# uzh-rpg/rpg_svo

Measured on AMD Instinct MI355X. Metric: frames/sec sparse-align+pose-refine (VGA, 4 pyr lvls); ATE vs CPU ref, higher is better.
Workload: dtype value = default build: K1 f32 pixels/residuals/chi2/per-pixel products, f64 Jacobian rows/partials/reductions/projection/solve/pose; K4 f64 (reference-width build: roofline_f64_build.value)

## Files before the change

### rpg_svo_amd/csrc/sparse_align.hip

```cpp
#include <cstdlib>
#include <map>
#include <mutex>
#include <utility>

#include "sia_common.h"

using namespace svo_capi;
using namespace svo_dev;
using namespace svo_sia;

namespace {

#define MINW(BLOCK) ((BLOCK) >= 256 ? 4 : 3)

#ifdef SIA_PROFILE
#define SIA_T() ((long long)__builtin_readcyclecounter())
#define SIA_ACC(k, t0, t1) prof[k] += (t1) - (t0)
#else
#define SIA_T() 0ll
#define SIA_ACC(k, t0, t1)
#endif

constexpr int MAX_WAVES = SVO_HIP_MAX_PATCHES / 64;

#if defined(SIA_F64_PARTIALS)
using sia_pix = double;
using sia_acc = double;
#undef MINW
#define MINW(BLOCK) 3
#else
using sia_pix = float;
using sia_acc = double;
#endif

struct SplitModel {
  double q[2][4], t[2][3];
};

struct SiaLds {
  SplitModel sm;
  double Rt[12];
  int sw_done, sw_stop, sw_nmeas, sw_cur, sw_old;
  double sw_chi2;
  double H[21];
  double Hinv[36];
  double A[36];
  sia_acc part[2][MAX_WAVES][8];
  int chg[2][MAX_WAVES];
  int xfail;
  sia_acc Hpart[MAX_WAVES][24];
  long long lo[SVO_HIP_MAX_LEVELS];
  int lw[SVO_HIP_MAX_LEVELS];
  int lh[SVO_HIP_MAX_LEVELS];
  int lp[SVO_HIP_MAX_LEVELS];
};
__shared__ SiaLds g_s;


template <int PARTS>
__device__ __forceinline__ void sia_rebuild_hinv(int lane, int nw, [[maybe_unused]] XChunk* xh, [[maybe_unused]] int part,
                                                 [[maybe_unused]] unsigned gen, [[maybe_unused]] int& xfail) {
  asm volatile("" : "+v"(lane));
#ifndef SVO_HOST_MATH_TEST
  if constexpr (PARTS > 1) {
    static_assert((PARTS - 1) * 21 <= 64, "one lane per chunk of the other parts");
    const int j = lane / 21, k = lane - 21 * j;
    double v = 0.0;
    for (int w = 0; w < nw; ++w) v += (double)g_s.Hpart[w][k];
    if (j == 0) sia_xstore(xh + part * SIA_XH_SLOTS + k, v, gen);
    const int other = j < part ? j : j + 1;
    double got = 0.0;
    if (j < PARTS - 1) got = sia_xpoll(xh + other * SIA_XH_SLOTS + k, gen, xfail);
    if (xfail) g_s.xfail = 1;
    double tot = 0.0;
#pragma unroll
    for (int p = 0; p < PARTS; ++p) {
      const double theirs = __shfl(got, (p < part ? p : p - 1) * 21 + k, 64);
      const double term = p == part ? v : theirs;
      tot = p == 0 ? term : tot + term;
    }
    if (lane < 21) g_s.H[lane] = tot;
  } else
#endif
  if (lane < 21) {
    double v = 0.0;
    for (int w = 0; w < nw; ++w) v += (double)g_s.Hpart[w][lane];
    g_s.H[lane] = v;
  }
  SVO_WAVE_LDS_FENCE();
  const int gi = lane / 6, gj = lane - 6 * gi;
  if (lane < 36) {
    g_s.A[lane] = g_s.H[sym6_rt(gi, gj)];
    g_s.Hinv[lane] = (gi == gj) ? 1.0 : 0.0;
  }
  for (int k = 0; k < 6; ++k) {
    SVO_WAVE_LDS_FENCE();
    if (lane < 36) {
      const double p = g_s.A[k * 6 + k];
      const double aik = g_s.A[gi * 6 + k];
      const double akj = g_s.A[k * 6 + gj];
      const double bkj = g_s.Hinv[k * 6 + gj];
      const double aij = g_s.A[lane];
      const double bij = g_s.Hinv[lane];
      const double ip = (fabs(p) > 2.2250738585072014e-308) ? sia_rcp(p) : 0.0;
      const double na = (gi == k) ? akj * ip : aij - aik * (akj * ip);
      const double nb = (gi == k) ? bkj * ip : bij - aik * (bkj * ip);
      SVO_LANES_LDS_FENCE();
      g_s.A[lane] = na;
      g_s.Hinv[lane] = nb;
    }
  }
}


__device__ __forceinline__ float sia_bilerp(float wtl, float wtr, float wbl, float wbr, float tl, float tr, float bl, float br) {
  return __builtin_fmaf(wbr, br, __builtin_fmaf(wbl, bl, __builtin_fmaf(wtr, tr, wtl * tl)));
}
typedef float sia_f2 __attribute__((ext_vector_type(2)));
__device__ __forceinline__ sia_f2 sia_bilerp2(sia_f2 wtl, sia_f2 wtr, sia_f2 wbl, sia_f2 wbr, sia_f2 tl, sia_f2 tr, sia_f2 bl,
                                              sia_f2 br) {
  return __builtin_elementwise_fma(wbr, br, __builtin_elementwise_fma(wbl, bl, __builtin_elementwise_fma(wtr, tr, wtl * tl)));
}

#ifdef SIA_F64_PARTIALS
#define SIA_PACKED 0
#else
#define SIA_PACKED 1
#endif
template <int BLOCK, bool WC, bool DIST, int PARTS = 1>
__global__ void __launch_bounds__(BLOCK, PARTS > 1 ? 1 : ((DIST && BLOCK < 1024) ? 3 : MINW(BLOCK))) sia_kernel(const SiaArgs a) {
  constexpr int NW = BLOCK / 64;
  int b, part = 0;
  if constexpr (PARTS > 1) {
    b = (int)(blockIdx.x / (8 * PARTS)) * 8 + (int)(blockIdx.x % 8);
    part = (int)(blockIdx.x / 8) % PARTS;
    if (b >= a.B) return;
  } else {
    b = (int)xcd_contiguous_block();
  }
  [[maybe_unused]] XChunk* const xbase = PARTS > 1 ? static_cast<XChunk*>(a.xw) + (size_t)b * SIA_X_BLOCK : nullptr;
  [[maybe_unused]] unsigned xseq = 0;
#ifndef SVO_HOST_MATH_TEST
  if constexpr (PARTS > 1) xseq = (unsigned)__builtin_amdgcn_readfirstlane((int)sia_xload(xbase + SIA_X_CHUNKS).lo);
#endif
  [[maybe_unused]] int xfail = 0;
  const int tid = threadIdx.x;
  const int lane = tid & 63;
  const int wave = tid >> 6;

  __shared__ float4 s_bt[8][BLOCK];

  int n = a.n[b];
  n = n > a.n_stride ? a.n_stride : n;
  const svo_hip_sia_params P = a.P;

  if (n <= 0) {
    if (tid == 0 && part == 0) {
      for (int k = 0; k < 12; ++k) a.T_out[12 * b + k] = a.T_in[12 * b + k];
      if (a.H_out)
        for (int k = 0; k < 36; ++k) a.H_out[36 * b + k] = 0.0;
      a.n_tracked[b] = 0;
      if (a.iters)
        for (int k = 0; k < SVO_HIP_MAX_LEVELS; ++k) a.iters[SVO_HIP_MAX_LEVELS * b + k] = 0;
      if (a.chi2) a.chi2[b] = 1e10;
      if (a.status) a.status[b] = 0;
    }
    return;
  }

  const int pid = part * BLOCK + tid;
  const size_t fo = (size_t)b * a.n_stride + pid;
  const bool has = (pid < n) && (a.valid ? a.valid[fo] != 0 : true);
  double X = 0, Y = 0, Z = 1;
  if (has) {
    X = a.xyz[3 * fo];
    Y = a.xyz[3 * fo + 1];
    Z = a.xyz[3 * fo + 2];
  }
  double px_kept0 = 0, px_kept1 = 0;
  if (has) {
    px_kept0 = a.px[2 * fo];
    px_kept1 = a.px[2 * fo + 1];
  }
  const double rz = sia_rcp(Z);
  const sia_acc zi = (sia_acc)rz;
  const sia_acc xn = (sia_acc)(X * rz);
  const sia_acc yn = (sia_acc)(Y * rz);
  const uint8_t* ref_base = a.store + (int64_t)a.ref_slot[b] * a.L.slot_bytes;
  const uint8_t* cur_base = a.store + (int64_t)a.cur_slot[b] * a.L.slot_bytes;

  if (tid == 0) {
#pragma unroll
    for (int k = 0; k < SVO_HIP_MAX_LEVELS; ++k) {
      g_s.lw[k] = a.L.w[k];
      g_s.lh[k] = a.L.h[k];
      g_s.lp[k] = a.L.pitch[k];
      g_s.lo[k] = a.L.offset[k];
    }
    for (int k = 0; k < 21; ++k) g_s.H[k] = 0.0;
    g_s.xfail = 0;
    if (a.iters && part == 0)
      for (int k = 0; k < SVO_HIP_MAX_LEVELS; ++k) a.iters[SVO_HIP_MAX_LEVELS * b + k] = 0;
  }
  double R[9], tr[3];
  {
    double q[4];
    for (int k = 0; k < 9; ++k) R[k] = a.T_in[12 * b + k];
    for (int k = 0; k < 3; ++k) tr[k] = a.T_in[12 * b + 9 + k];
    quat_from_R(R, q);
    quat_to_R(q, R);
    if (tid == 0) {
      for (int k = 0; k < 4; ++k) g_s.sm.q[0][k] = q[k];
      for (int k = 0; k < 3; ++k) g_s.sm.t[0][k] = tr[k];
    }
  }
  int m_cur = 0, m_old = 0;
  double chi2_prev = 1e10;
  int stop = 0;
  int n_meas_last = 0;
  int buf = 0;

  const int sw = (NW > 1) ? (int)(blockIdx.x % NW) : 0;
  sia_pix Sxx = 0, Sxy = 0, Syy = 0;
  sia_acc gmask = 0;
  bool vis = false;

  __syncthreads();

#ifdef SIA_PROFILE
  long long prof[8] = {0, 0, 0, 0, 0, 0, 0, 0};
  const long long t_begin = SIA_T();
#endif
  for (int level = P.max_level; level >= P.min_level; --level) {
    [[maybe_unused]] const long long tl0 = SIA_T();
    const int cols = g_s.lw[level], rows = g_s.lh[level], pitch = g_s.lp[level];
    const uint8_t* ref_img = ref_base + g_s.lo[level];
    const uint8_t* cur_img = cur_base + g_s.lo[level];
    const float scale = pow2_inv_f32(level);
    const sia_acc fl = (sia_acc)(fabs(P.fx) * pow2_inv_f64(level));

    uint32_t wc[WC ? 7 : 1][3];
    int wc_u0 = 0, wc_v0 = -100000;
    if (WC) {
#pragma unroll
      for (int r = 0; r < (WC ? 7 : 1); ++r) wc[r][0] = wc[r][1] = wc[r][2] = 0u;
    }
    {
      const double pxx = px_kept0, pxy = px_kept1;
      const float u_ref = (float)(pxx * (double)scale);
      const float v_ref = (float)(pxy * (double)scale);
      const int u_i = (int)floorf(u_ref);
      const int v_i = (int)floorf(v_ref);
      const bool inb = has && !(u_i - 3 < 0 || v_i - 3 < 0 || u_i + 3 >= cols || v_i + 3 >= rows);
      Sxx = Sxy = Syy = 0;
      if (inb) {
        vis = true;
        gmask = 1;
        const float su = u_ref - (float)u_i, sv = v_ref - (float)v_i;
        const float wtl = (1.f - su) * (1.f - sv);
        const float wtr = su * (1.f - sv);
        const float wbl = (1.f - su) * sv;
        const float wbr = su * sv;
        float Bt[6][6];
        float Wp[7], Wc[7];
        uint32_t rw[7][3];
        const int rxa = run_start(u_i - 3, 7);
        const uint32_t rbo = (uint32_t)(u_i - 3 - rxa);
        load_window12<7>(ref_img, pitch, rxa, v_i - 3, rw);
        cut_row7(rw[0], rbo, Wp);
#pragma unroll
        for (int r = 0; r < 6; ++r) {
          cut_row7(rw[r + 1], rbo, Wc);
#pragma unroll
          for (int c = 0; c < 6; ++c) {
            const bool need = ((r >= 1 && r <= 4)) || ((c >= 1 && c <= 4));
            if (need) Bt[r][c] = sia_bilerp(wtl, wtr, wbl, wbr, Wp[c], Wp[c + 1], Wc[c], Wc[c + 1]);
          }
#pragma unroll
          for (int c = 0; c < 7; ++c) Wp[c] = Wc[c];
        }
#pragma unroll
        for (int y = 0; y < 4; ++y)
#pragma unroll
          for (int x = 0; x < 4; ++x) {
            const float dx = 0.5f * (Bt[y + 1][x + 2] - Bt[y + 1][x]);
            const float dy = 0.5f * (Bt[y + 2][x + 1] - Bt[y][x + 1]);
            Sxx += (sia_pix)dx * (sia_pix)dx;
            Sxy += (sia_pix)dx * (sia_pix)dy;
            Syy += (sia_pix)dy * (sia_pix)dy;
          }
#if SIA_PACKED
        s_bt[0][tid] = make_float4(Bt[0][1], Bt[0][3], Bt[0][2], Bt[0][4]);
        s_bt[1][tid] = make_float4(Bt[1][0], Bt[1][2], Bt[1][1], Bt[1][3]);
        s_bt[2][tid] = make_float4(Bt[1][4], Bt[1][5], Bt[2][0], Bt[2][2]);
        s_bt[3][tid] = make_float4(Bt[2][1], Bt[2][3], Bt[2][4], Bt[2][5]);
        s_bt[4][tid] = make_float4(Bt[3][0], Bt[3][2], Bt[3][1], Bt[3][3]);
        s_bt[5][tid] = make_float4(Bt[3][4], Bt[3][5], Bt[4][0], Bt[4][2]);
        s_bt[6][tid] = make_float4(Bt[4][1], Bt[4][3], Bt[4][4], Bt[4][5]);
        s_bt[7][tid] = make_float4(Bt[5][1], Bt[5][3], Bt[5][2], Bt[5][4]);
#else
        s_bt[0][tid] = make_float4(Bt[0][1], Bt[0][2], Bt[0][3], Bt[0][4]);
        s_bt[1][tid] = make_float4(Bt[1][0], Bt[1][1], Bt[1][2], Bt[1][3]);
        s_bt[2][tid] = make_float4(Bt[1][4], Bt[1][5], Bt[2][0], Bt[2][1]);
        s_bt[3][tid] = make_float4(Bt[2][2], Bt[2][3], Bt[2][4], Bt[2][5]);
        s_bt[4][tid] = make_float4(Bt[3][0], Bt[3][1], Bt[3][2], Bt[3][3]);
        s_bt[5][tid] = make_float4(Bt[3][4], Bt[3][5], Bt[4][0], Bt[4][1]);
        s_bt[6][tid] = make_float4(Bt[4][2], Bt[4][3], Bt[4][4], Bt[4][5]);
        s_bt[7][tid] = make_float4(Bt[5][1], Bt[5][2], Bt[5][3], Bt[5][4]);
#endif
      } else {
        gmask = 0;
      }
    }

    m_old = m_cur;
    int inH = -1;
    int evals = 0;
    SIA_ACC(5, tl0, SIA_T());
    for (int iter = 0; iter < P.n_iter; ++iter) {
      [[maybe_unused]] const long long tp0 = SIA_T();
      bool m = false;
      sia_pix gx = 0, gy = 0;
      float c2 = 0.f;
      if (vis) {
        const double xc = R[0] * X + R[1] * Y + R[2] * Z + tr[0];
        const double yc = R[3] * X + R[4] * Y + R[5] * Z + tr[1];
        const double zc = R[6] * X + R[7] * Y + R[8] * Z + tr[2];
        double izc = __builtin_amdgcn_rcp(zc);
        izc = fma(fma(-zc, izc, 1.0), izc, izc);
        izc = fma(fma(-zc, izc, 1.0), izc, izc);
        double pu, pv;
        if (DIST) {
          Cam cm;
          cm.fx = P.fx; cm.fy = P.fy; cm.cx = P.cx; cm.cy = P.cy;
          cm.width = 0; cm.height = 0;
          cm.model = P.cam_model;
#pragma unroll
          for (int k = 0; k < 5; ++k) cm.d[k] = P.d[k];
          const double uvn[2] = {xc * izc, yc * izc};
          double pxd[2];
          world2cam_uv(cm, uvn, pxd);
          pu = pxd[0];
          pv = pxd[1];
        } else {
          pu = P.fx * (xc * izc) + P.cx;
          pv = P.fy * (yc * izc) + P.cy;
        }
        const float u_cur = (float)pu * scale;
        const float v_cur = (float)pv * scale;
        const float fu = floorf(u_cur), fv = floorf(v_cur);
        if (fu - 3.f >= 0.f && fv - 3.f >= 0.f && fu + 3.f < (float)cols && fv + 3.f < (float)rows) {
          m = true;
          const int u_i = (int)fu, v_i = (int)fv;
          const float su = u_cur - fu, sv = v_cur - fv;
          const float wtl = (1.f - su) * (1.f - sv);
          const float wtr = su * (1.f - sv);
          const float wbl = (1.f - su) * sv;
          const float wbr = su * sv;
          {
#if SIA_PACKED
          typedef float f2 __attribute__((ext_vector_type(2)));
          uint32_t cw[5][3];
          uint32_t cbo = 0;
          uint64_t k0 = 0, k1 = 0, kup = 0;
          int bo = 0;
          if (WC) {
            int r0 = (v_i - 2) - wc_v0;
            bo = (u_i - 2) - wc_u0;
            if (!(r0 >= 0 && r0 <= 2 && bo >= 0 && bo <= 7)) {
              wc_v0 = v_i - 3;
              wc_u0 = run_start(u_i - 3, 7);
              load_window12<(WC ? 7 : 1)>(cur_img, pitch, wc_u0, wc_v0, wc);
              r0 = 1;
              bo = (u_i - 2) - wc_u0;
            }
            k0 = SVO_BALLOT_ACTIVE(r0 == 0);
            k1 = SVO_BALLOT_ACTIVE(r0 == 1);
            kup = SVO_BALLOT_ACTIVE(bo >= 4);
          } else {
            const int cxa = run_start(u_i - 2, 5);
            cbo = (uint32_t)(u_i - 2 - cxa);
            load_window12<5>(cur_img, pitch, cxa, v_i - 2, cw);
          }
#define SIA_WIN_ROW(r, p02, p13, p24)                                                                                   \
  do {                                                                                                                  \
    float o_[5];                                                                                                        \
    if (WC) {                                                                                                           \
      constexpr int S_ = WC ? 1 : 0;                                                                                    \
      const uint32_t d0_ = sel_e64(k0, wc[(r) * S_][0], sel_e64(k1, wc[((r) + 1) * S_][0], wc[((r) + 2) * S_][0]));     \
      const uint32_t d1_ = sel_e64(k0, wc[(r) * S_][1], sel_e64(k1, wc[((r) + 1) * S_][1], wc[((r) + 2) * S_][1]));     \
      const uint32_t d2_ = sel_e64(k0, wc[(r) * S_][2], sel_e64(k1, wc[((r) + 1) * S_][2], wc[((r) + 2) * S_][2]));     \
      cut_row5(d0_, d1_, d2_, bo, kup, o_);                                                                             \
    } else {                                                                                                            \
      cut_row5_plain(cw[WC ? 0 : (r)], cbo, o_);                                                                        \
    }                                                                                                                   \
    p02 = f2{o_[0], o_[2]};                                                                                             \
    p13 = f2{o_[1], o_[3]};                                                                                             \
    p24 = f2{o_[2], o_[4]};                                                                                             \
  } while (0)
          const float2* const bt2 = reinterpret_cast<const float2*>(&s_bt[0][0]);
#define SIA_BT2(q, h) bt2[((q) * BLOCK + tid) * 2 + (h)]
          const f2 vtl = f2{wtl, wtl}, vtr = f2{wtr, wtr}, vbl = f2{wbl, wbl}, vbr = f2{wbr, wbr};
          f2 c2v = f2{0.f, 0.f}, gxv = f2{0.f, 0.f}, gyv = f2{0.f, 0.f};
          f2 t02, t13, t24, b02, b13, b24;
          SIA_WIN_ROW(0, t02, t13, t24);
          SIA_WIN_ROW(1, b02, b13, b24);
          f2 a13, a24, b02t, b13t, b45t, c02, c13, c45;
          { const float2 v0 = SIA_BT2(0, 0), v1 = SIA_BT2(0, 1); a13 = f2{v0.x, v0.y}; a24 = f2{v1.x, v1.y}; }
          { const float2 v0 = SIA_BT2(1, 0), v1 = SIA_BT2(1, 1), v2 = SIA_BT2(2, 0);
            b02t = f2{v0.x, v0.y}; b13t = f2{v1.x, v1.y}; b45t = f2{v2.x, v2.y}; }
          { const float2 v0 = SIA_BT2(2, 1), v1 = SIA_BT2(3, 0), v2 = SIA_BT2(3, 1);
            c02 = f2{v0.x, v0.y}; c13 = f2{v1.x, v1.y}; c45 = f2{v2.x, v2.y}; }
#pragma unroll
          for (int y = 0; y < 4; ++y) {
            f2 n02 = f2{0.f, 0.f}, n13 = f2{0.f, 0.f}, n45 = f2{0.f, 0.f};
            if (y == 0) { const float2 v0 = SIA_BT2(4, 0), v1 = SIA_BT2(4, 1), v2 = SIA_BT2(5, 0);
                          n02 = f2{v0.x, v0.y}; n13 = f2{v1.x, v1.y}; n45 = f2{v2.x, v2.y}; }
            if (y == 1) { const float2 v0 = SIA_BT2(5, 1), v1 = SIA_BT2(6, 0), v2 = SIA_BT2(6, 1);
                          n02 = f2{v0.x, v0.y}; n13 = f2{v1.x, v1.y}; n45 = f2{v2.x, v2.y}; }
            if (y == 2) { const float2 v0 = SIA_BT2(7, 0), v1 = SIA_BT2(7, 1);
                          n13 = f2{v0.x, v0.y}; n45 = f2{v1.x, v1.y}; }
            const f2 b24t = f2{b02t.y, b45t.x}, b35t = f2{b13t.y, b45t.y};
            const f2 c24 = (y < 3) ? f2{c02.y, c45.x} : c45;
            const f2 Ia = sia_bilerp2(vtl, vtr, vbl, vbr, t02, t13, b02, b13);
            const f2 Ib = sia_bilerp2(vtl, vtr, vbl, vbr, t13, t24, b13, b24);
            const f2 ra = Ia - b13t, rb = Ib - b24t;
            c2v += ra * ra;
            c2v += rb * rb;
            gxv += ra * (b24t - b02t);
            gxv += rb * (b35t - b13t);
            gyv += ra * (c13 - a13);
            gyv += rb * (c24 - a24);
            if (y < 3) {
              f2 w02, w13, w24;
              SIA_WIN_ROW(y + 2, w02, w13, w24);
              t02 = b02; t13 = b13; t24 = b24;
              b02 = w02; b13 = w13; b24 = w24;
              a13 = b13t; a24 = b24t;
              b02t = c02; b13t = c13; b45t = c45;
              c02 = n02; c13 = n13; c45 = n45;
              asm volatile("" ::: "memory");
            }
          }
#undef SIA_WIN_ROW
#undef SIA_BT2
          c2 += c2v.x + c2v.y;
          gx += gxv.x + gxv.y;
          gy += gyv.x + gyv.y;
#else
          float W[5][5];
          if (WC) {
            int r0 = (v_i - 2) - wc_v0;
            int bo = (u_i - 2) - wc_u0;
            if (!(r0 >= 0 && r0 <= 2 && bo >= 0 && bo <= 7)) {
              wc_v0 = v_i - 3;
              wc_u0 = run_start(u_i - 3, 7);
              load_window12<(WC ? 7 : 1)>(cur_img, pitch, wc_u0, wc_v0, wc);
              r0 = 1;
              bo = (u_i - 2) - wc_u0;
            }
            const uint64_t k0 = SVO_BALLOT_ACTIVE(r0 == 0), k1 = SVO_BALLOT_ACTIVE(r0 == 1);
            const uint64_t kup = SVO_BALLOT_ACTIVE(bo >= 4);
#pragma unroll
            for (int r = 0; r < 5; ++r) {
              constexpr int S = WC ? 1 : 0;
              const uint32_t d0 = sel_e64(k0, wc[r * S][0], sel_e64(k1, wc[(r + 1) * S][0], wc[(r + 2) * S][0]));
              const uint32_t d1 = sel_e64(k0, wc[r * S][1], sel_e64(k1, wc[(r + 1) * S][1], wc[(r + 2) * S][1]));
              const uint32_t d2 = sel_e64(k0, wc[r * S][2], sel_e64(k1, wc[(r + 1) * S][2], wc[(r + 2) * S][2]));
              cut_row5(d0, d1, d2, bo, kup, W[r]);
            }
          } else {
            uint32_t cw[5][3];
            const int cxa = run_start(u_i - 2, 5);
            const uint32_t cbo = (uint32_t)(u_i - 2 - cxa);
            load_window12<5>(cur_img, pitch, cxa, v_i - 2, cw);
#pragma unroll
            for (int r = 0; r < 5; ++r) cut_row5_plain(cw[r], cbo, W[r]);
          }
          float Bt[6][6];
          {
            const float4 q0 = s_bt[0][tid], q1 = s_bt[1][tid], q2 = s_bt[2][tid], q3 = s_bt[3][tid];
            const float4 q4 = s_bt[4][tid], q5 = s_bt[5][tid], q6 = s_bt[6][tid], q7 = s_bt[7][tid];
            Bt[0][0] = Bt[0][5] = Bt[5][0] = Bt[5][5] = 0.f;
            Bt[0][1] = q0.x; Bt[0][2] = q0.y; Bt[0][3] = q0.z; Bt[0][4] = q0.w;
            Bt[1][0] = q1.x; Bt[1][1] = q1.y; Bt[1][2] = q1.z; Bt[1][3] = q1.w;
            Bt[1][4] = q2.x; Bt[1][5] = q2.y; Bt[2][0] = q2.z; Bt[2][1] = q2.w;
            Bt[2][2] = q3.x; Bt[2][3] = q3.y; Bt[2][4] = q3.z; Bt[2][5] = q3.w;
            Bt[3][0] = q4.x; Bt[3][1] = q4.y; Bt[3][2] = q4.z; Bt[3][3] = q4.w;
            Bt[3][4] = q5.x; Bt[3][5] = q5.y; Bt[4][0] = q5.z; Bt[4][1] = q5.w;
            Bt[4][2] = q6.x; Bt[4][3] = q6.y; Bt[4][4] = q6.z; Bt[4][5] = q6.w;
            Bt[5][1] = q7.x; Bt[5][2] = q7.y; Bt[5][3] = q7.z; Bt[5][4] = q7.w;
          }
#pragma unroll
          for (int y = 0; y < 4; ++y)
#pragma unroll
            for (int x = 0; x < 4; ++x) {
              const float I = sia_bilerp(wtl, wtr, wbl, wbr, W[y][x], W[y][x + 1], W[y + 1][x], W[y + 1][x + 1]);
              const float res = I - Bt[y + 1][x + 1];
              c2 += res * res;
              gx += (sia_pix)res * (sia_pix)(Bt[y + 1][x + 2] - Bt[y + 1][x]);
              gy += (sia_pix)res * (sia_pix)(Bt[y + 2][x + 1] - Bt[y][x + 1]);
            }
#endif
          }
        }
      }
      {
        const sia_acc gsc = (sia_acc)0.5 * fl * gmask;
        const sia_acc gxf = m ? (sia_acc)gx * gsc : (sia_acc)0, gyf = m ? (sia_acc)gy * gsc : (sia_acc)0;
        sia_acc part[8];
        sia_acc zi_ = zi, xn_ = xn, yn_ = yn;
        asm volatile("" : "+v"(zi_), "+v"(xn_), "+v"(yn_));
        part[0] = zi_ * gxf;
        part[1] = zi_ * gyf;
        part[2] = -zi_ * (xn_ * gxf + yn_ * gyf);
        part[3] = -(xn_ * yn_ * gxf + ((sia_acc)1 + yn_ * yn_) * gyf);
        part[4] = ((sia_acc)1 + xn_ * xn_) * gxf + xn_ * yn_ * gyf;
        part[5] = xn_ * gyf - yn_ * gxf;
        part[6] = (sia_acc)c2;
        part[7] = m ? (sia_acc)16 : (sia_acc)0;
        [[maybe_unused]] const long long tp1 = SIA_T();
        SIA_ACC(0, tp0, tp1);
        const sia_acc tot = wave_reduce8(part, lane);
        if ((lane & 7) == 0) g_s.part[buf][wave][lane >> 3] = tot;
        const int mine = __builtin_amdgcn_ballot_w64((int)m != inH) != 0ull;
        if (lane == 0) g_s.chg[buf][wave] = mine;
        SIA_ACC(1, tp1, SIA_T());
      }
      [[maybe_unused]] const long long tb0 = SIA_T();
      __syncthreads();
      int changed = 0;
#pragma unroll
      for (int w = 0; w < NW; ++w) changed |= g_s.chg[buf][w];
      [[maybe_unused]] double xtot = 0.0;
#ifndef SVO_HOST_MATH_TEST
      if constexpr (PARTS > 1) {
        ++xseq;
        const int xp = lane >> 4, xk = lane & 15;
        double own = 0.0;
        if (xk < 8) {
#pragma unroll
          for (int w = 0; w < NW; ++w) own += (double)g_s.part[buf][w][xk];
        } else if (xk == 8) {
          own = (double)changed;
        }
        XChunk* const slot = xbase + (size_t)(xseq & 1) * (SIA_X_MAX_PARTS * SIA_X_SLOTS);
        if (wave == sw && xp == part && xk < 9) sia_xstore(slot + part * SIA_X_SLOTS + xk, own, xseq);
        double val = own;
        if (xp != part && xp < PARTS && xk < 9) val = sia_xpoll(slot + xp * SIA_X_SLOTS + xk, xseq, xfail);
        if (xfail) g_s.xfail = 1;
        xtot = __shfl(val, xk, 64);
#pragma unroll
        for (int p = 1; p < PARTS; ++p) xtot += __shfl(val, 16 * p + xk, 64);
        changed = readlane_f64<8>(xtot) != 0.0;
      }
#endif
      [[maybe_unused]] const long long tb1 = SIA_T();
      SIA_ACC(2, tb0, tb1);
      if (changed) {
        sia_acc zi_ = zi, xn_ = xn, yn_ = yn;
        asm volatile("" : "+v"(zi_), "+v"(xn_), "+v"(yn_));
        const sia_acc one = 1, zero = 0;
        const sia_acc ja[6] = {-zi_ * fl, zero, xn_ * zi_ * fl, xn_ * yn_ * fl, -(one + xn_ * xn_) * fl, yn_ * fl};
        const sia_acc jb[6] = {zero, -zi_ * fl, yn_ * zi_ * fl, (one + yn_ * yn_) * fl, -xn_ * yn_ * fl, -xn_ * fl};
        sia_acc hp[24];
#pragma unroll
        for (int i = 0; i < 6; ++i)
#pragma unroll
          for (int j = i; j < 6; ++j) {
            const sia_acc v = (sia_acc)Sxx * (ja[i] * ja[j]) + (sia_acc)Sxy * (ja[i] * jb[j] + jb[i] * ja[j]) + (sia_acc)Syy * (jb[i] * jb[j]);
            hp[sym6(i, j)] = m ? v : zero;
          }
        hp[21] = hp[22] = hp[23] = zero;
#pragma unroll
        for (int g = 0; g < 3; ++g) {
          const sia_acc tot = wave_reduce8(hp + 8 * g, lane);
          if ((lane & 7) == 0) g_s.Hpart[wave][8 * g + (lane >> 3)] = tot;
        }
        inH = (int)m;
        __syncthreads();
        if constexpr (PARTS > 1) {
          ++xseq;
          XChunk* const xh = xbase + 2 * SIA_X_MAX_PARTS * SIA_X_SLOTS + (size_t)(xseq & 1) * (SIA_X_MAX_PARTS * SIA_XH_SLOTS);
          if (wave == 0) sia_rebuild_hinv<PARTS>(lane, NW, xh, part, xseq, xfail);
        } else {
          if (wave == 0) sia_rebuild_hinv<1>(lane, NW, nullptr, 0, 0u, xfail);
        }
        __syncthreads();
      }
      ++evals;
      [[maybe_unused]] const long long ts0 = SIA_T();
      SIA_ACC(3, tb1, ts0);
#ifdef SIA_PROFILE
      prof[7] += 1;
#endif

      int done = 0;
      const int swb = (NW > 1) ? (sw + 1) % NW : sw;
      const bool rot_wave = wave == sw, trans_wave = wave == swb;
      int m_next = m_cur;
      if (rot_wave || trans_wave) {
        __builtin_amdgcn_s_setprio(3);
        double colsum = 0.0;
        if constexpr (PARTS > 1) {
          colsum = xtot;
        } else {
          const int k = lane & 7;
#pragma unroll
          for (int w = 0; w < NW; ++w) colsum += (double)g_s.part[buf][w][k];
        }
        const double b0 = readlane_f64<0>(colsum), b1 = readlane_f64<1>(colsum), b2 = readlane_f64<2>(colsum);
        const double b3 = readlane_f64<3>(colsum), b4 = readlane_f64<4>(colsum), b5 = readlane_f64<5>(colsum);
        const float chi2_sum = (float)readlane_f64<6>(colsum);
        const int n_meas = (int)readlane_f64<7>(colsum);
        double xi;
        {
          const double* row = &g_s.Hinv[6 * (lane < 6 ? lane : 0)];
          xi = row[0] * b0 + row[1] * b1 + row[2] * b2 + row[3] * b3 + row[4] * b4 + row[5] * b5;
        }
        const double x0 = readlane_f64<0>(xi), x1 = readlane_f64<1>(xi), x2 = readlane_f64<2>(xi);
        const double x3 = readlane_f64<3>(xi), x4 = readlane_f64<4>(xi), x5 = readlane_f64<5>(xi);
        n_meas_last = n_meas;
        const double new_chi2 = (double)(chi2_sum / (float)n_meas);
        if (isnan(x0)) stop = 1;
        const SplitModel& sm = g_s.sm;
        const bool rollback = (iter > 0 && new_chi2 > chi2_prev) || stop;
        if (rollback) {
          m_next = m_old;
          done = 1;
        } else {
          m_next = m_cur ^ 1;
          m_old = m_cur;
          chi2_prev = new_chi2;
          const double nm = fmax(fmax(fmax(fabs(x0), fabs(x1)), fmax(fabs(x2), fabs(x3))), fmax(fabs(x4), fabs(x5)));
          if (nm <= P.eps) done = 1;
        }
        const float mx[6] = {-(float)x0, -(float)x1, -(float)x2, -(float)x3, -(float)x4, -(float)x5};
        if (rot_wave) {
          double q[4];
          if (rollback) {
#pragma unroll
            for (int k = 0; k < 4; ++k) q[k] = sm.q[m_next][k];
          } else {
#ifdef SIA_F64_PARTIALS
            const double mxd[6] = {-x0, -x1, -x2, -x3, -x4, -x5};
            double eq[4], et_unused[3];
            se3_exp(mxd, eq, et_unused);
#else
            float eqf[4];
            se3_exp_rot_f32(mx, eqf);
            const double eq[4] = {eqf[0], eqf[1], eqf[2], eqf[3]};
#endif
            double oq[4];
#pragma unroll
            for (int k = 0; k < 4; ++k) oq[k] = sm.q[m_cur][k];
            quat_mul(oq, eq, q);
            quat_normalize_fast(q);
            if (lane == 0) {
#pragma unroll
              for (int k = 0; k < 4; ++k) g_s.sm.q[m_next][k] = q[k];
            }
          }
          quat_to_R(q, R);
          if (lane == 0) {
#pragma unroll
            for (int k = 0; k < 9; ++k) g_s.Rt[k] = R[k];
            g_s.sw_done = done;
            g_s.sw_stop = stop;
            g_s.sw_nmeas = n_meas_last;
            g_s.sw_chi2 = chi2_prev;
            g_s.sw_cur = m_next;
            g_s.sw_old = m_old;
          }
        }
        if (trans_wave) {
          if (rollback) {
#pragma unroll
            for (int k = 0; k < 3; ++k) tr[k] = sm.t[m_next][k];
          } else {
#ifdef SIA_F64_PARTIALS
            const double mxd[6] = {-x0, -x1, -x2, -x3, -x4, -x5};
            double eq_unused[4], et[3];
            se3_exp(mxd, eq_unused, et);
#else
            float etf[3];
            se3_exp_trans_f32(mx, etf);
            const double et[3] = {etf[0], etf[1], etf[2]};
#endif
            double oq[4], rt[3];
#pragma unroll
            for (int k = 0; k < 4; ++k) oq[k] = sm.q[m_cur][k];
            quat_rot(oq, et, rt);
#pragma unroll
            for (int k = 0; k < 3; ++k) tr[k] = sm.t[m_cur][k] + rt[k];
            if (lane == 0) {
#pragma unroll
              for (int k = 0; k < 3; ++k) g_s.sm.t[m_next][k] = tr[k];
            }
          }
          if (lane == 0) {
#pragma unroll
            for (int k = 0; k < 3; ++k) g_s.Rt[9 + k] = tr[k];
          }
        }
        __builtin_amdgcn_s_setprio(0);
      }
      m_cur = m_next;
      if (NW > 1) {
        __syncthreads();
#pragma unroll
        for (int k = 0; k < 9; ++k) R[k] = g_s.Rt[k];
#pragma unroll
        for (int k = 0; k < 3; ++k) tr[k] = g_s.Rt[9 + k];
        done = g_s.sw_done;
        stop = g_s.sw_stop;
        n_meas_last = g_s.sw_nmeas;
        chi2_prev = g_s.sw_chi2;
        m_cur = g_s.sw_cur;
        m_old = g_s.sw_old;
      }
      buf ^= 1;
      SIA_ACC(4, ts0, SIA_T());
      if (done) break;
    }
    if (tid == 0 && part == 0 && a.iters) a.iters[SVO_HIP_MAX_LEVELS * b + level] = evals;
  }

  if (tid == 0 && part == 0) {
    for (int k = 0; k < 9; ++k) a.T_out[12 * b + k] = R[k];
    for (int k = 0; k < 3; ++k) a.T_out[12 * b + 9 + k] = tr[k];
    if (a.H_out)
      for (int i = 0; i < 6; ++i)
        for (int j = 0; j < 6; ++j) a.H_out[36 * b + i * 6 + j] = g_s.H[sym6_rt(i, j)];
#ifdef SIA_PROFILE
    prof[6] = SIA_T() - t_begin;
    if (a.H_out)
      for (int k = 0; k < 8; ++k) a.H_out[36 * b + k] = (double)prof[k];
#endif
    a.n_tracked[b] = n_meas_last / 16;
    if (a.chi2) a.chi2[b] = chi2_prev;
    if constexpr (PARTS > 1) {
#ifndef SVO_HOST_MATH_TEST
      sia_xstore_epoch(xbase + SIA_X_CHUNKS, xseq + (g_s.xfail ? (1u << 16) : 0u));
#endif
    }
    if (a.status) a.status[b] = (stop ? SVO_HIP_SIA_STOP : 0) | ((PARTS > 1 && g_s.xfail) ? SVO_HIP_SIA_EXCHANGE_TIMEOUT : 0);
  }
}


template <int BLOCK>
int launch(const SiaArgs& args, int B, hipStream_t s) {
  constexpr bool WC = BLOCK == 256;
  if (args.P.cam_model == SVO_HIP_CAM_PINHOLE)
    hipLaunchKernelGGL((sia_kernel<BLOCK, WC, false>), dim3(B), dim3(BLOCK), 0, s, args);
  else
    hipLaunchKernelGGL((sia_kernel<BLOCK, false, true>), dim3(B), dim3(BLOCK), 0, s, args);
  return check_launch();
}

}

namespace {

int sia_prepare(const svo_hip_pyr_layout* layout, const uint8_t* d_store, int B, const int32_t* d_ref_slot,
                const int32_t* d_cur_slot, const int32_t* d_n, int n_stride, const double* d_px, const double* d_xyz_ref,
                const uint8_t* d_valid, const svo_hip_sia_params* params, const double* d_T_in, double* d_T_out,
                double* d_H_out, int32_t* d_n_tracked, int32_t* d_iters, double* d_chi2, int32_t* d_status, SiaArgs* out) {
  if (!layout_ok(layout) || !d_store || !params || B < 0) return SVO_HIP_EINVAL;
  if (B == 0) return SVO_HIP_OK;
  if (!d_ref_slot || !d_cur_slot || !d_n || !d_px || !d_xyz_ref || !d_T_in || !d_T_out || !d_n_tracked)
    return SVO_HIP_EINVAL;
  if (n_stride < 1) return SVO_HIP_EINVAL;
  if (n_stride > SVO_HIP_MAX_PATCHES) return SVO_HIP_ERANGE;
  if (params->min_level < 0 || params->max_level < params->min_level || params->max_level >= layout->n_levels ||
      params->n_iter < 0)
    return SVO_HIP_EINVAL;
  if (params->cam_model != SVO_HIP_CAM_PINHOLE && params->cam_model != SVO_HIP_CAM_PINHOLE_RADTAN &&
      params->cam_model != SVO_HIP_CAM_ATAN)
    return SVO_HIP_EINVAL;
  SiaArgs& args = *out;
  args.L = *layout;
  args.store = d_store;
  args.ref_slot = d_ref_slot;
  args.cur_slot = d_cur_slot;
  args.n = d_n;
  args.n_stride = n_stride;
  args.px = d_px;
  args.xyz = d_xyz_ref;
  args.valid = d_valid;
  args.P = *params;
  args.T_in = d_T_in;
  args.T_out = d_T_out;
  args.H_out = d_H_out;
  args.n_tracked = d_n_tracked;
  args.iters = d_iters;
  args.chi2 = d_chi2;
  args.status = d_status;
  return 1;
}

constexpr int SIA_SPLIT_PARTS = 4;
constexpr int SIA_SPLIT_MAX_B = 128;
#ifndef SVO_HOST_MATH_TEST
bool sia_split_applies(const SiaArgs& args, int B) {
  static const bool on = [] { const char* v = std::getenv("SVO_HIP_K1_SPLIT"); return !(v && v[0] == '0'); }();
  return on && args.n_stride > 512 && B <= SIA_SPLIT_MAX_B;
}
void* sia_split_blocks(hipStream_t s) {
  static std::mutex mut;
  static std::map<std::pair<int, hipStream_t>, void*> blocks;
  int dev = 0;
  if (hipGetDevice(&dev) != hipSuccess) return nullptr;
  std::lock_guard<std::mutex> g(mut);
  void*& p = blocks[std::make_pair(dev, s)];
  if (p) return p;
  hipStreamCaptureStatus cap = hipStreamCaptureStatusNone;
  if (hipStreamIsCapturing(s, &cap) != hipSuccess || cap != hipStreamCaptureStatusNone) return nullptr;
  const size_t bytes = (size_t)SIA_SPLIT_MAX_B * SIA_X_BLOCK * sizeof(XChunk);
  void* q = nullptr;
  if (hipMalloc(&q, bytes) != hipSuccess) return nullptr;
  if (hipMemset(q, 0, bytes) != hipSuccess || hipDeviceSynchronize() != hipSuccess) {
    (void)hipFree(q);
    return nullptr;
  }
  p = q;
  return p;
}
int launch_split(SiaArgs args, int B, void* xw, hipStream_t s) {
  args.B = B;
  args.xw = xw;
  const dim3 grid((unsigned)((B + 7) / 8) * 8 * SIA_SPLIT_PARTS), blk(256);
  if (args.P.cam_model == SVO_HIP_CAM_PINHOLE)
    hipLaunchKernelGGL((sia_kernel<256, true, false, SIA_SPLIT_PARTS>), grid, blk, 0, s, args);
  else
    hipLaunchKernelGGL((sia_kernel<256, false, true, SIA_SPLIT_PARTS>), grid, blk, 0, s, args);
  return check_launch();
}
#endif

int launch_workgroup(const SiaArgs& args, int B, hipStream_t s) {
  if (args.n_stride <= 64) return launch<64>(args, B, s);
  if (args.n_stride <= 128) return launch<128>(args, B, s);
  if (args.n_stride <= 256) return launch<256>(args, B, s);
  if (args.n_stride <= 512) return launch<512>(args, B, s);
  return launch<1024>(args, B, s);
}

}

extern "C" int svo_hip_sparse_align(const svo_hip_pyr_layout* layout, const uint8_t* d_store, int B,
                                    const int32_t* d_ref_slot, const int32_t* d_cur_slot, const int32_t* d_n,
                                    int n_stride, const double* d_px, const double* d_xyz_ref,
                                    const uint8_t* d_valid, const svo_hip_sia_params* params,
                                    const double* d_T_in, double* d_T_out, double* d_H_out,
                                    int32_t* d_n_tracked, int32_t* d_iters, double* d_chi2, int32_t* d_status,
                                    void* stream) {
  SiaArgs args;
  const int rc = sia_prepare(layout, d_store, B, d_ref_slot, d_cur_slot, d_n, n_stride, d_px, d_xyz_ref, d_valid, params,
                             d_T_in, d_T_out, d_H_out, d_n_tracked, d_iters, d_chi2, d_status, &args);
  if (rc <= 0) return rc;
  hipStream_t s = static_cast<hipStream_t>(stream);
  if (sia_wave_applies(args, B)) return launch_sia_wave(args, B, s);
#ifndef SVO_HOST_MATH_TEST
  if (sia_split_applies(args, B))
    if (void* xw = sia_split_blocks(s)) return launch_split(args, B, xw, s);
#endif
  return launch_workgroup(args, B, s);
}

extern "C" int svo_hip_sparse_align_workgroup(const svo_hip_pyr_layout* layout, const uint8_t* d_store, int B,
                                              const int32_t* d_ref_slot, const int32_t* d_cur_slot, const int32_t* d_n,
                                              int n_stride, const double* d_px, const double* d_xyz_ref,
                                              const uint8_t* d_valid, const svo_hip_sia_params* params,
                                              const double* d_T_in, double* d_T_out, double* d_H_out,
                                              int32_t* d_n_tracked, int32_t* d_iters, double* d_chi2,
                                              int32_t* d_status, void* stream) {
  SiaArgs args;
  const int rc = sia_prepare(layout, d_store, B, d_ref_slot, d_cur_slot, d_n, n_stride, d_px, d_xyz_ref, d_valid, params,
                             d_T_in, d_T_out, d_H_out, d_n_tracked, d_iters, d_chi2, d_status, &args);
  if (rc <= 0) return rc;
  return launch_workgroup(args, B, static_cast<hipStream_t>(stream));
}
```

Before: 11.54 million.

## Compute Hessian before barrier and invert redundantly in both solver waves

For the single-part windowed-cache path, per-wave Hessian partials are now built before the shared barrier, and only when that wave's inlier ballot changed. The 6x6 inverse is rebuilt by both the rotation and translation waves into separate LDS copies, which removes the extra barrier after the Hessian stage. The LDS layout is templated on wave count to shrink shared memory, and the current-frame window load is issued early, overlapped with the reference patch setup. The cost is duplicated inversion work, extra LDS for the second copy, and more code complexity.

```diff
diff --git a/rpg_svo_amd/csrc/sparse_align.hip b/rpg_svo_amd/csrc/sparse_align.hip
--- a/rpg_svo_amd/csrc/sparse_align.hip
+++ b/rpg_svo_amd/csrc/sparse_align.hip
@@ -37,7 +37,15 @@
   double q[2][4], t[2][3];
 };
 
-struct SiaLds {
+template <bool TWO>
+struct SiaLdsOwn {};
+template <>
+struct SiaLdsOwn<true> {
+  double A2[36], Hinv2[36];
+};
+
+template <int LW, bool TWO>
+struct SiaLdsT : SiaLdsOwn<TWO> {
   SplitModel sm;
   double Rt[12];
   int sw_done, sw_stop, sw_nmeas, sw_cur, sw_old;
@@ -45,16 +53,24 @@
   double H[21];
   double Hinv[36];
   double A[36];
-  sia_acc part[2][MAX_WAVES][8];
-  int chg[2][MAX_WAVES];
+  sia_acc part[2][LW][8];
+  int chg[2][LW];
   int xfail;
-  sia_acc Hpart[MAX_WAVES][24];
+  sia_acc Hpart[LW][24];
   long long lo[SVO_HIP_MAX_LEVELS];
   int lw[SVO_HIP_MAX_LEVELS];
   int lh[SVO_HIP_MAX_LEVELS];
   int lp[SVO_HIP_MAX_LEVELS];
 };
+using SiaLds = SiaLdsT<MAX_WAVES, false>;
 __shared__ SiaLds g_s;
+template <int LW>
+__shared__ SiaLdsT<LW, (LW > 1)> g_ls;
+template <bool LS, int NW>
+__device__ __forceinline__ auto& sia_lds() {
+  if constexpr (LS) return g_ls<NW>;
+  else return g_s;
+}
 
 
 template <int PARTS>
@@ -112,6 +128,63 @@
   }
 }
 
+template <int NR>
+__device__ __forceinline__ void sia_window12_issue(const uint8_t* __restrict__ lvl, int pitch, int xa, int v0, uint32_t d[][3]) {
+  const uint32_t c = svo_pyr::col_off(xa);
+  const int o = xa & 15;
+  const uint32_t o8 = o == 12 ? 116u : 0u;
+  const uint32_t o4 = o <= 4 ? 8u : (o == 8 ? 120u : 0u);
+#pragma unroll
+  for (int r = 0; r < NR; ++r) {
+    const uint32_t a = svo_pyr::row_off(v0 + r, pitch) + c;
+    const svo_pyr::u32x2_t v = svo_pyr::ld64(lvl, a + o8);
+    d[r][0] = v.x; d[r][1] = v.y;
+    d[r][2] = svo_pyr::ld32(lvl, a + o4);
+  }
+}
+template <int NR>
+__device__ __forceinline__ void sia_window12_order(int xa, uint32_t d[][3]) {
+  const bool late8 = (xa & 15) == 12;
+#pragma unroll
+  for (int r = 0; r < NR; ++r) {
+    const uint32_t p0 = d[r][0], p1 = d[r][1], p2 = d[r][2];
+    d[r][0] = late8 ? p2 : p0;
+    d[r][1] = late8 ? p0 : p1;
+    d[r][2] = late8 ? p1 : p2;
+  }
+}
+
+__device__ __forceinline__ void sia_own_hinv(int nw, const sia_acc (*Hpart)[24], double* H, double* A, double* Hinv) {
+  const int lane = (int)__builtin_amdgcn_mbcnt_hi(~0u, __builtin_amdgcn_mbcnt_lo(~0u, 0u));
+  const int gi = lane / 6, gj = lane - 6 * gi;
+  if (lane < 36) {
+    const int e = sym6_rt(gi, gj);
+    double v = 0.0;
+    for (int w = 0; w < nw; ++w) v += (double)Hpart[w][e];
+    if (H && gi <= gj) H[e] = v;
+    A[lane] = v;
+    Hinv[lane] = (gi == gj) ? 1.0 : 0.0;
+  }
+  for (int k = 0; k < 6; ++k) {
+    SVO_WAVE_LDS_FENCE();
+    if (lane < 36) {
+      const double p = A[k * 6 + k];
+      const double aik = A[gi * 6 + k];
+      const double akj = A[k * 6 + gj];
+      const double bkj = Hinv[k * 6 + gj];
+      const double aij = A[lane];
+      const double bij = Hinv[lane];
+      const double ip = (fabs(p) > 2.2250738585072014e-308) ? sia_rcp(p) : 0.0;
+      const double na = (gi == k) ? akj * ip : aij - aik * (akj * ip);
+      const double nb = (gi == k) ? bkj * ip : bij - aik * (bkj * ip);
+      SVO_LANES_LDS_FENCE();
+      A[lane] = na;
+      Hinv[lane] = nb;
+    }
+  }
+  SVO_WAVE_LDS_FENCE();
+}
+
 
 __device__ __forceinline__ float sia_bilerp(float wtl, float wtr, float wbl, float wbr, float tl, float tr, float bl, float br) {
   return __builtin_fmaf(wbr, br, __builtin_fmaf(wbl, bl, __builtin_fmaf(wtr, tr, wtl * tl)));
@@ -130,6 +203,8 @@
 template <int BLOCK, bool WC, bool DIST, int PARTS = 1>
 __global__ void __launch_bounds__(BLOCK, PARTS > 1 ? 1 : ((DIST && BLOCK < 1024) ? 3 : MINW(BLOCK))) sia_kernel(const SiaArgs a) {
   constexpr int NW = BLOCK / 64;
+  constexpr bool LS = PARTS == 1 && WC;
+  auto& g_s = sia_lds<LS, NW>();
   int b, part = 0;
   if constexpr (PARTS > 1) {
     b = (int)(blockIdx.x / (8 * PARTS)) * 8 + (int)(blockIdx.x % 8);
@@ -146,7 +221,7 @@
   [[maybe_unused]] int xfail = 0;
   const int tid = threadIdx.x;
   const int lane = tid & 63;
-  const int wave = tid >> 6;
+  const int wave = LS ? __builtin_amdgcn_readfirstlane(tid >> 6) : tid >> 6;
 
   __shared__ float4 s_bt[8][BLOCK];
 
@@ -253,6 +328,24 @@
       const int v_i = (int)floorf(v_ref);
       const bool inb = has && !(u_i - 3 < 0 || v_i - 3 < 0 || u_i + 3 >= cols || v_i + 3 >= rows);
       Sxx = Sxy = Syy = 0;
+      if constexpr (LS) {
+        if ((vis || inb) && P.n_iter > 0) {
+          const double xc = R[0] * X + R[1] * Y + R[2] * Z + tr[0];
+          const double yc = R[3] * X + R[4] * Y + R[5] * Z + tr[1];
+          const double zc = R[6] * X + R[7] * Y + R[8] * Z + tr[2];
+          double izc = __builtin_amdgcn_rcp(zc);
+          izc = fma(fma(-zc, izc, 1.0), izc, izc);
+          izc = fma(fma(-zc, izc, 1.0), izc, izc);
+          const double pu = P.fx * (xc * izc) + P.cx;
+          const double pv = P.fy * (yc * izc) + P.cy;
+          const float fu = floorf((float)pu * scale), fv = floorf((float)pv * scale);
+          if (fu - 3.f >= 0.f && fv - 3.f >= 0.f && fu + 3.f < (float)cols && fv + 3.f < (float)rows) {
+            wc_v0 = (int)fv - 3;
+            wc_u0 = run_start((int)fu - 3, 7);
+            sia_window12_issue<(WC ? 7 : 1)>(cur_img, pitch, wc_u0, wc_v0, wc);
+          }
+        }
+      }
       if (inb) {
         vis = true;
         gmask = 1;
@@ -311,10 +404,13 @@
       } else {
         gmask = 0;
       }
+      if constexpr (LS) sia_window12_order<(WC ? 7 : 1)>(wc_u0, wc);
     }
 
     m_old = m_cur;
     int inH = -1;
+    [[maybe_unused]] unsigned long long h_in = 0ull;
+    [[maybe_unused]] bool h_have = false;
     int evals = 0;
     SIA_ACC(5, tl0, SIA_T());
     for (int iter = 0; iter < P.n_iter; ++iter) {
@@ -505,6 +601,12 @@
           }
         }
       }
+      [[maybe_unused]] unsigned long long h_now = 0ull;
+      [[maybe_unused]] bool h_renew = false;
+      if constexpr (LS) {
+        h_now = __builtin_amdgcn_ballot_w64(m);
+        h_renew = !h_have || h_now != h_in;
+      }
       {
         const sia_acc gsc = (sia_acc)0.5 * fl * gmask;
         const sia_acc gxf = m ? (sia_acc)gx * gsc : (sia_acc)0, gyf = m ? (sia_acc)gy * gsc : (sia_acc)0;
@@ -522,10 +624,42 @@
         [[maybe_unused]] const long long tp1 = SIA_T();
         SIA_ACC(0, tp0, tp1);
         const sia_acc tot = wave_reduce8(part, lane);
-        if ((lane & 7) == 0) g_s.part[buf][wave][lane >> 3] = tot;
-        const int mine = __builtin_amdgcn_ballot_w64((int)m != inH) != 0ull;
+        int lane_w = lane;
+        if constexpr (LS) {
+          lane_w = (int)__builtin_amdgcn_mbcnt_hi(~0u, __builtin_amdgcn_mbcnt_lo(~0u, 0u));
+          asm volatile("" : "+v"(lane_w));
+        }
+        if ((lane & 7) == 0) g_s.part[buf][wave][lane_w >> 3] = tot;
+        const int mine = LS ? (int)h_renew : (int)(__builtin_amdgcn_ballot_w64((int)m != inH) != 0ull);
         if (lane == 0) g_s.chg[buf][wave] = mine;
         SIA_ACC(1, tp1, SIA_T());
+      }
+      if constexpr (LS) {
+        [[maybe_unused]] const long long th0 = SIA_T();
+        if (h_renew) {
+          sia_acc zi_ = zi, xn_ = xn, yn_ = yn;
+          asm volatile("" : "+v"(zi_), "+v"(xn_), "+v"(yn_));
+          const sia_acc one = 1, zero = 0;
+          const sia_acc ja[6] = {-zi_ * fl, zero, xn_ * zi_ * fl, xn_ * yn_ * fl, -(one + xn_ * xn_) * fl, yn_ * fl};
+          const sia_acc jb[6] = {zero, -zi_ * fl, yn_ * zi_ * fl, (one + yn_ * yn_) * fl, -xn_ * yn_ * fl, -xn_ * fl};
+          sia_acc hp[24];
+#pragma unroll
+          for (int i = 0; i < 6; ++i)
+#pragma unroll
+            for (int j = i; j < 6; ++j) {
+              const sia_acc v = (sia_acc)Sxx * (ja[i] * ja[j]) + (sia_acc)Sxy * (ja[i] * jb[j] + jb[i] * ja[j]) + (sia_acc)Syy * (jb[i] * jb[j]);
+              hp[sym6(i, j)] = m ? v : zero;
+            }
+          hp[21] = hp[22] = hp[23] = zero;
+#pragma unroll
+          for (int g = 0; g < 3; ++g) {
+            const sia_acc tot = wave_reduce8(hp + 8 * g, lane);
+            if ((lane & 7) == 0) g_s.Hpart[wave][8 * g + (lane >> 3)] = tot;
+          }
+          h_in = h_now;
+          h_have = true;
+        }
+        SIA_ACC(3, th0, SIA_T());
       }
       [[maybe_unused]] const long long tb0 = SIA_T();
       __syncthreads();
@@ -557,7 +691,7 @@
 #endif
       [[maybe_unused]] const long long tb1 = SIA_T();
       SIA_ACC(2, tb0, tb1);
-      if (changed) {
+      if (!LS && changed) {
         sia_acc zi_ = zi, xn_ = xn, yn_ = yn;
         asm volatile("" : "+v"(zi_), "+v"(xn_), "+v"(yn_));
         const sia_acc one = 1, zero = 0;
@@ -601,6 +735,22 @@
       int m_next = m_cur;
       if (rot_wave || trans_wave) {
         __builtin_amdgcn_s_setprio(3);
+        [[maybe_unused]] const double* hinv = g_s.Hinv;
+        if constexpr (LS) {
+          [[maybe_unused]] const long long tr0 = SIA_T();
+          if constexpr (NW > 1) {
+            if (!rot_wave) hinv = g_s.Hinv2;
+            if (changed) {
+              if (rot_wave) sia_own_hinv(NW, g_s.Hpart, g_s.H, g_s.A, g_s.Hinv);
+              else sia_own_hinv(NW, g_s.Hpart, nullptr, g_s.A2, g_s.Hinv2);
+            }
+          } else {
+            if (changed) sia_own_hinv(NW, g_s.Hpart, g_s.H, g_s.A, g_s.Hinv);
+          }
+          [[maybe_unused]] const long long tr1 = SIA_T();
+          SIA_ACC(3, tr0, tr1);
+          SIA_ACC(4, tr1, tr0);
+        }
         double colsum = 0.0;
         if constexpr (PARTS > 1) {
           colsum = xtot;
@@ -615,7 +765,7 @@
         const int n_meas = (int)readlane_f64<7>(colsum);
         double xi;
         {
-          const double* row = &g_s.Hinv[6 * (lane < 6 ? lane : 0)];
+          const double* row = &(LS ? hinv : g_s.Hinv)[6 * (lane < 6 ? lane : 0)];
           xi = row[0] * b0 + row[1] * b1 + row[2] * b2 + row[3] * b3 + row[4] * b4 + row[5] * b5;
         }
         const double x0 = readlane_f64<0>(xi), x1 = readlane_f64<1>(xi), x2 = readlane_f64<2>(xi);
```

Result: slower. 11.16 million (-3.3%).
